# xds0112/5G_based_System_level_Integrated_Sensing_and_Communication_Simulator

Hardware: AMD Instinct MI355X
Metric: sensing slots/sec (CDL echo->2D-FFT->2D-CFAR) (higher is better)
Workload: dtype f64

## Files before the change

### 5g_based_system_level_integrated_sensing_and_communication_simulator_amd/csrc/cov.hip

```cpp
#include <algorithm>
#include <type_traits>
#include "isac_internal.hpp"
#include "echo_dev.hpp"

namespace isac {

typedef double v4f64 __attribute__((ext_vector_type(4)));


constexpr int kCovSyncSlabs = 8;
template <int NB>
struct CovPlan {
  static constexpr int kTiles = NB * (NB + 1) / 2;
  static constexpr int kGroups = (kTiles + 4) / 5;
  static constexpr int kPerGroup = (kTiles + kGroups - 1) / kGroups;
  static constexpr int kPhases = 4 / kGroups;
  static constexpr int kSamplesPerLane = 4 / kPhases;
  static constexpr int first_tile(int grp) { return grp * kPerGroup; }
  static constexpr int tiles_of(int grp) { return first_tile(grp) + kPerGroup <= kTiles ? kPerGroup : kTiles - first_tile(grp); }
};

constexpr int cov_tile_i(int nb, int t) {
  int i = 0;
  while (t >= nb - i) { t -= nb - i; ++i; }
// ... 610 lines not shown
  unsigned long long seed;
  int K, L_whole, L_out, A;
  int s_col;
};
constexpr int kLazyPieces = 19;
__host__ __device__ constexpr int lazy_piece_gap(int i) {
  return (i * 30) / kLazyPieces;
}

template <int QT>
struct CovLazyGenerator {
  static constexpr int NB = 4;
  static constexpr int kGaps = 30;
  struct Cur { int l, sc; long long g; };
  int gp, ga, K, s_col, g_lds0;
  double sig;
  uint32_t key0, key1;
  long long s_end;
  c64 st[2][QT];
  bool ant_ok[2];
  uint64_t colbase[2];
  __amdgpu_buffer_rsrc_t rsD[QT];
  Cur cg, cd;
  uint32_t pc[2][4];
  float wf[2][2][2];
  bool v_half[2];
  c64 dl[2][QT][2];
  __device__ __forceinline__ CovLazyGenerator(const LazyCovArgs& a, long long s_begin, long long s_end_)
      : gp(threadIdx.x & 7), ga(threadIdx.x >> 3), K(a.K), s_col(a.s_col), sig(a.sig), key0((uint32_t)a.seed), key1((uint32_t)(a.seed >> 32)), s_end(s_end_) {
#pragma unroll
    for (int j = 0; j < 2; ++j) {
      const int ant = ga + 32 * j;
      ant_ok[j] = ant < a.A;
      colbase[j] = (uint64_t)a.L_out * (uint64_t)ant;
#pragma unroll
      for (int q = 0; q < QT; ++q) st[j][q] = ant_ok[j] ? a.steer_rq[(long long)ant * QT + q] : mk(0.0, 0.0);
    }
#pragma unroll
    for (int q = 0; q < QT; ++q) rsD[q] = buffer_of(a.D + (long long)q * K * a.L_whole, (unsigned)((long long)K * a.L_whole * (long long)sizeof(c64)));
    g_lds0 = (ga >> 4) * kCovSlabBlk + gp * kCovPitch + ((ga & 15) ^ kCovSwizzle(gp));
    cg = cd = cur_at(s_begin);
  }
  __device__ __forceinline__ Cur cur_at(long long g) const {
    Cur c; c.g = g; c.l = (int)((unsigned)g / (unsigned)s_col); c.sc = (int)((unsigned)g - (unsigned)c.l * (unsigned)s_col); return c;
  }
  __device__ __forceinline__ void advance(Cur& c) const { ++c.g; if (++c.sc == s_col) { c.sc = 0; ++c.l; } }
  __device__ __forceinline__ int k0_of(const Cur& c) const { return ((c.sc >> 6) << 10) + ((c.sc & 63) << 3) + gp; }
  __device__ __forceinline__ void init(const Cur& c) {
    const int k0 = k0_of(c);
    const bool in = c.g < s_end;
    v_half[0] = in && k0 < K;
    v_half[1] = in && k0 + 512 < K;
    const uint32_t slot = (uint32_t)(((c.sc >> 6) << 9) + ((c.sc & 63) << 3) + gp);
#pragma unroll
    for (int j = 0; j < 2; ++j) {
      const uint64_t ctr = (uint64_t)slot + (uint64_t)kSpectralSlotsPerColumn * ((uint64_t)c.l + colbase[j]);
      pc[j][0] = (uint32_t)ctr; pc[j][1] = (uint32_t)(ctr >> 32); pc[j][2] = kSpectralStream; pc[j][3] = 0u;
    }
  }
  template <int R>
  __device__ __forceinline__ void round() {
#pragma unroll
    for (int j = 0; j < 2; ++j) philox4x32_round(pc[j], key0 + (uint32_t)R * 0x9E3779B9u, key1 + (uint32_t)R * 0xBB67AE85u);
  }
  template <int I>
  __device__ __forceinline__ void bm() {
    constexpr int j = I / 2, h = I % 2;
    box_muller32_hw_f32(pc[j][2 * h], pc[j][2 * h + 1], wf[j][h][0], wf[j][h][1]);
  }
  template <int I>
  __device__ __forceinline__ void emit(const c64 (&dv)[QT][2], c64* img) {
    constexpr int j = I / 2, h = I % 2;
    c64 d[QT];
#pragma unroll
    for (int q = 0; q < QT; ++q) d[q] = dv[q][h];
    c64 v = spectral_echo_value<QT, true>(d, st[j], mk((double)wf[j][h][0], (double)wf[j][h][1]), sig);
    const bool ok = v_half[h] && ant_ok[j];
    v = mk(ok ? v.re : 0.0, ok ? v.im : 0.0);
    img[g_lds0 + 2 * j * kCovSlabBlk + 8 * h * kCovPitch] = v;
  }
  __device__ __forceinline__ void loads(c64 (&dv)[QT][2], const Cur& c) {
    const int k0 = k0_of(c);
    const bool in = c.g < s_end;
    const unsigned base = (unsigned)(((long long)K * c.l + k0) * (long long)sizeof(c64));
    const unsigned o0 = (in && k0 < K) ? base : kCovOobOffset, o1 = (in && k0 + 512 < K) ? base + 512u * (unsigned)sizeof(c64) : kCovOobOffset;
#pragma unroll
    for (int q = 0; q < QT; ++q) { dv[q][0] = buffer_load_c64(rsD[q], o0); dv[q][1] = buffer_load_c64(rsD[q], o1); }
  }
  __device__ __forceinline__ void whole(c64 (&dv)[QT][2], c64* img) {
// ... 294 lines not shown
```

### 5g_based_system_level_integrated_sensing_and_communication_simulator_amd/csrc/echo.hip

```cpp
#include <cstring>
#include <type_traits>

#include "isac_internal.hpp"
#include "fft_lds.hpp"
#include "echo_dev.hpp"

namespace isac {

template <int QT, int UNROLL>
__global__ __launch_bounds__(256) void beamsum_kernel(const c64* __restrict__ tx, long long T, int A,
                                                      const c64* __restrict__ steer ,
                                                      c64* __restrict__ beam ) {
  extern __shared__ __attribute__((aligned(16))) char smem_raw[];
  c64* s_steer = reinterpret_cast<c64*>(smem_raw);
  for (int i = threadIdx.x; i < A * QT; i += blockDim.x) s_steer[i] = steer[i];
  __syncthreads();
  for (long long t0 = (long long)blockIdx.x * 256; t0 < T; t0 += (long long)gridDim.x * 256) {
    const long long t = t0 + threadIdx.x;
    const long long tc = t < T ? t : T - 1;
    c64 acc[QT];
#pragma unroll
    for (int q = 0; q < QT; ++q) acc[q] = mk(0.0, 0.0);
    const c64* p = tx + tc;
    int a = 0;
    for (; a + UNROLL <= A; a += UNROLL) {
      c64 v[UNROLL];
#pragma unroll
      for (int u = 0; u < UNROLL; ++u) v[u] = p[(long long)(a + u) * T];
#pragma unroll
      for (int u = 0; u < UNROLL; ++u)
#pragma unroll
        for (int q = 0; q < QT; ++q) acc[q] = fma(v[u], s_steer[q * A + a + u], acc[q]);
    }
    for (; a < A; ++a) {
      c64 v = p[(long long)a * T];
#pragma unroll
      for (int q = 0; q < QT; ++q) acc[q] = fma(v, s_steer[q * A + a], acc[q]);
    }
    if (t < T) {
#pragma unroll
      for (int q = 0; q < QT; ++q) beam[(long long)q * T + t] = acc[q];
    }
  }
}

struct TargetDesc {
  double wd;
  double lsf;
  long long shift;
};
constexpr int kMaxTargets = 64;
struct TargetTable {
  TargetDesc t[kMaxTargets];
};

__global__ __launch_bounds__(256) void coef_kernel(const c64* __restrict__ beam, long long T, int Q,
                                                   TargetTable tab, double w , double Ts,
                                                   c64* __restrict__ coef ,
                                                   c64* __restrict__ phase_rx ) {
  long long t = (long long)blockIdx.x * blockDim.x + threadIdx.x;
  if (t >= T) return;
  double tt = (double)t * Ts;
  double s, c;
  sincos(w * tt, &s, &c);
  c64 prx = mk(c, -s);
  phase_rx[t] = prx;
  for (int q = 0; q < Q; ++q) {
    long long d = tab.t[q].shift;
    c64 out = mk(0.0, 0.0);
    if (t >= d) {
      double sd, cd, st, ct;
      sincos(tab.t[q].wd * tt, &sd, &cd);
      sincos(w * ((double)(t - d) * Ts), &st, &ct);
      c64 v = beam[(long long)q * T + (t - d)] * mk(ct, st);
      v = v * mk(cd, sd);
      v = v * tab.t[q].lsf;
      out = v * prx;
    }
    coef[(long long)q * T + t] = out;
  }
}

__global__ __launch_bounds__(256) void radar_waveform_kernel(long long T, int A, int Q, const c64* __restrict__ coef,
                                                             const c64* __restrict__ steer_rq ,
                                                             const c64* __restrict__ phase_rx, int noise_mode,
                                                             const c64* __restrict__ noise, double n0s, uint64_t seed,
                                                             c64* __restrict__ rx) {
  long long t = (long long)blockIdx.x * blockDim.x + threadIdx.x;
  int r = blockIdx.y;
  if (t >= T) return;
  rx[t + T * r] = rx_sample(t, r, T, Q, coef, steer_rq + (long long)r * Q, phase_rx, noise_mode, noise, n0s, seed);
}

struct OfdmGeom {
  int nfft, n_sc, cp_base, cp_long, sym_per_half;
};

template <class FFT, bool SYNTH, int QT = 0>
__global__ __launch_bounds__(256, 2) void demod_kernel(OfdmGeom g, long long T, int A, int L_whole, int L_out,
                                                       const c64* __restrict__ tw,
                                                       int Q_rt, const c64* __restrict__ coef,
                                                       const c64* __restrict__ steer_rq, const c64* __restrict__ phase_rx,
                                                       int noise_mode, const c64* __restrict__ noise, double n0s,
                                                       uint64_t seed,
                                                       const c64* __restrict__ wave,
                                                       c64* __restrict__ grid, const c64* __restrict__ logtab_g) {
  extern __shared__ __attribute__((aligned(16))) char smem_raw[];
  c64* lds = reinterpret_cast<c64*>(smem_raw);
  const int tid = threadIdx.x;
  FFT fft;
  constexpr bool kTables = SYNTH && QT > 0 && std::is_same<FFT, Fft4096>::value;
  const int Q = QT ? QT : Q_rt;
// ... 127 lines not shown
template <int QT, int NZ, bool STORE = true, int GROUP = (QT <= 1 ? 4 : 2)>
__global__ __launch_bounds__(Fft4096W::NT, kEchoRangeWavesPerSimd) void echo_range_sl_kernel(int K, int L_whole, int L_out, int A, const c64* D,
                                                            const c64* __restrict__ steer_rq, double sig, uint64_t seed,
                                                            const c64* noise, const c64* __restrict__ tw,
                                                            c64* grid,
                                                            const c64* txg, const double* win_k,
                                                            const double* __restrict__ win_r, double inv_n, double sqrt_n,
                                                            int row_lo, int n_rows, c64* __restrict__ ymid) {
  static_assert(QT >= 1 && QT <= 2, "compile-time target count");
  extern __shared__ __attribute__((aligned(16))) char smem_raw[];
  c64* lds = reinterpret_cast<c64*>(smem_raw);
  using FFT = Fft4096W;
  constexpr int NT = FFT::NT, PER = FFT::PER, NG = PER / GROUP;
  const int tid = threadIdx.x;
  FFT fft;
  int l, r;
  if (!spectral_tile_map(blockIdx.x, L_whole, A, l, r)) return;
  const long long colg = (long long)l + (long long)L_out * r;
  const c64* Dl = D + (long long)K * l;
  const long long d_stride = (long long)K * L_whole;
  const c64* ptx = txg + (long long)K * colg;
  const c64* nzc = NZ == 2 ? noise + (long long)K * colg : nullptr;
  const __amdgpu_buffer_rsrc_t rs_dst = buffer_of(grid + (long long)K * colg, (unsigned)K * (unsigned)sizeof(c64));
  c64 s[QT];
#pragma unroll
  for (int q = 0; q < QT; ++q) s[q] = steer_rq[(long long)r * QT + q];
  struct Ld { c64 tx; double w; c64 d[QT]; c64 nz; };
  Ld ld[2][GROUP];
  auto load_group = [&](int g, int b) {
#pragma unroll
    for (int u = 0; u < GROUP; ++u) {
      const int k = tid + NT * (g * GROUP + u);
      const int kc = k < K ? k : K - 1;
      Ld& e = ld[b][u];
      e.tx = ptx[kc];
      e.w = win_k[kc];
      if constexpr (NZ == 2) e.nz = nzc[kc];
#pragma unroll
      for (int q = 0; q < QT; ++q) e.d[q] = Dl[(long long)q * d_stride + kc];
    }
    asm volatile("" ::: "memory");
  };
  fft.init_table(lds, tw, tid);
  load_group(0, 0);
  __builtin_amdgcn_sched_barrier(0);
#pragma unroll
  for (int j = 0; j < PER; ++j) fft.x[j] = mk(0.0, 0.0);
  const int wave_k0 = __builtin_amdgcn_readfirstlane(tid & ~63);
  auto draw = [&](int c) {
    if constexpr (NZ == 1) {
      const int j0 = 2 * c, j1 = j0 + 1;
      if (wave_k0 + NT * j0 < K) {
        const uint64_t ctr = (uint64_t)(tid + NT * c) + (uint64_t)kSpectralSlotsPerColumn * (uint64_t)colg;
        uint32_t o[4];
        philox4x32_10((uint32_t)ctr, (uint32_t)(ctr >> 32), kSpectralStream, 0u, (uint32_t)seed, (uint32_t)(seed >> 32), o);
        fft.x[j0] = box_muller32_hw(o[0], o[1]);
        if (wave_k0 + NT * j1 < K) fft.x[j1] = box_muller32_hw(o[2], o[3]);
      }
    }
  };
  bool live = false;
  auto consume = [&](int g, int b) {
#pragma unroll
    for (int u = 0; u < GROUP; ++u) {
      const int j = g * GROUP + u, k = tid + NT * j;
      const Ld& e = ld[b][u];
      const c64 v = spectral_echo_value<QT, NZ != 0>(e.d, s, NZ == 2 ? e.nz : fft.x[j], sig);
      if constexpr (STORE) buffer_store_c64_nt(rs_dst, (unsigned)k * (unsigned)sizeof(c64), v);
      else asm volatile("" ::"v"(v.re), "v"(v.im) : "memory");
      c64 y = mul_conj(v, e.tx) * e.w;
      y = k < K ? y : mk(0.0, 0.0);
      live |= (y.re != 0.0) | (y.im != 0.0);
      fft.x[j] = y;
    }
  };
#pragma unroll
  for (int g = 0; g < NG; ++g) {
#pragma unroll
    for (int c = g * GROUP / 2; c < (g + 1) * GROUP / 2; ++c) draw(c);
    __builtin_amdgcn_sched_barrier(0);
    if (g + 1 < NG) load_group(g + 1, (g + 1) & 1);
    consume(g, g & 1);
    __builtin_amdgcn_sched_barrier(0);
  }
  c64* yd = ymid + (long long)n_rows * colg;
  if (!__syncthreads_or(live)) {
    for (int rr = tid; rr < n_rows; rr += NT) yd[rr] = mk(0.0, 0.0);
    return;
  }
  fft.init_twiddles_lds(lds, tid);
  const int blk = FFT::block_of_rows(row_lo, n_rows);
  fft.template transform<+1>(lds, tw, tid, blk);
  auto put = [&](int n, c64 v) {
    const int rr = n - row_lo;
    const double wr = win_r[n];
    if (rr >= 0 && rr < n_rows) yd[rr] = ((v * inv_n) * sqrt_n) * wr;
  };
  if (blk >= 0) fft.drain_block(put, tid, blk);
  else fft.drain(put, tid);
}

struct ModIo {
  long long wave_rows, t_off;
  int grid_cols, l_off, sym0, n_win;
// ... 91 lines not shown
  if (c->scs_khz != 15 && c->scs_khz != 30 && c->scs_khz != 60 && c->scs_khz != 120)
    return fail(ctx, ISAC_ERR_INVALID_ARG, "carrier.scs_khz must be 15/30/60/120");
  return ISAC_OK;
}

static OfdmGeom geom_of(const isac_carrier* c) {
  Numerology n = numerology(c->nfft, c->scs_khz);
  return OfdmGeom{c->nfft, c->n_sc, n.cp_base, n.cp_long, n.sym_per_half};
}

static int whole_symbols(const OfdmGeom& g, long long T) {
  long long lo = 0, hi = T / g.nfft + 1;
  while (lo < hi) {
    long long mid = (lo + hi + 1) / 2;
    if (symbol_start((int)mid, g.nfft, g.cp_base, g.cp_long, g.sym_per_half) <= T) lo = mid; else hi = mid - 1;
  }
  return (int)lo;
}

extern "C" int isac_ofdm_symbol_count(const isac_carrier* carrier, int64_t T, int32_t* n_symbols) {
  if (!carrier || !n_symbols || T < 0) return ISAC_ERR_INVALID_ARG;
  *n_symbols = whole_symbols(geom_of(carrier), T);
  return ISAC_OK;
}

extern "C" int isac_ofdm_waveform_length(const isac_carrier* carrier, int32_t L, int64_t* T) {
  if (!carrier || !T || L < 0) return ISAC_ERR_INVALID_ARG;
  OfdmGeom g = geom_of(carrier);
  *T = symbol_start(L, g.nfft, g.cp_base, g.cp_long, g.sym_per_half);
  return ISAC_OK;
}

static int prepare_echo(isac_ctx* ctx, const c64* d_tx, long long T, const isac_radar_channel_params* rp,
                        const uint8_t* los, int* q_out) {
  if (!d_tx || !rp || !los) return fail(ctx, ISAC_ERR_INVALID_ARG, "NULL argument");
  if (T <= 0 || rp->n_ants <= 0 || rp->n_targets < 0) return fail(ctx, ISAC_ERR_INVALID_ARG, "bad T / n_ants / n_targets");
  ctx->lazy.valid = false;
  if (!(rp->fs > 0)) return fail(ctx, ISAC_ERR_INVALID_ARG, "fs must be positive");
  const int A = rp->n_ants;
  const double c0 = 299792458.0;
  const double lambda = c0 / rp->fc;
  const double Ts = 1.0 / rp->fs;
  const double two_pi = 2.0 * M_PI;
  TargetTable tab{};
  std::vector<c64> steer_aq;
  int Q = 0;
  for (int i = 0; i < rp->n_targets; ++i) {
    if (los[i] != 1) continue;
    if (Q >= kMaxTargets) return fail(ctx, ISAC_ERR_CAPACITY, "more than 64 LoS targets");
    for (int a = 0; a < A; ++a) {
      const isac_c64 sv = rp->rx_steering[(size_t)a + (size_t)A * i];
      steer_aq.push_back(mk(sv.re, sv.im));
    }
    double path_delay = 2.0 * rp->range[i] / c0;
    tab.t[Q].shift = (long long)std::ceil(path_delay / Ts);
    double fd = 2.0 * rp->velocity[i] / lambda;
    tab.t[Q].wd = two_pi * fd;
    tab.t[Q].lsf = rp->large_scale_fading[i];
    ++Q;
  }
  if (Q == 0) return fail(ctx, ISAC_ERR_NO_LOS, "no LoS target: rxWaveform is empty (basicRadarChannel.m:59,64)");
  std::vector<c64> steer_rq((size_t)A * Q);
  for (int q = 0; q < Q; ++q)
    for (int a = 0; a < A; ++a) steer_rq[(size_t)a * Q + q] = steer_aq[(size_t)q * A + a];
  ISAC_TRY(ensure(ctx, ctx->steer, sizeof(c64) * (size_t)A * Q * 2));
  ISAC_TRY(ensure(ctx, ctx->beam, sizeof(c64) * (size_t)Q * T));
  ISAC_TRY(ensure(ctx, ctx->coef, sizeof(c64) * (size_t)Q * T));
  ISAC_TRY(ensure(ctx, ctx->phase_rx, sizeof(c64) * (size_t)T));
  c64* d_steer_aq = (c64*)ctx->steer.p;
  {
    const size_t bytes = sizeof(c64) * (size_t)A * Q * 2;
    void* hst = nullptr;
    ISAC_TRY(stage_acquire(ctx, bytes, &hst));
    std::memcpy(hst, steer_aq.data(), bytes / 2);
    std::memcpy((char*)hst + bytes / 2, steer_rq.data(), bytes / 2);
    ISAC_TRY(stage_commit(ctx, d_steer_aq, bytes));
  }
  const unsigned gb = cdiv(T, 256);
  const unsigned gbs = (unsigned)std::min<long long>(gb, 1024);
  timeline_mark(ctx, 0, ctx->stream);
#define ISAC_BEAMSUM(QT) \
  hipLaunchKernelGGL((beamsum_kernel<QT, (QT <= 2 ? 32 : 8)>), dim3(gbs), dim3(256), sizeof(c64) * A * QT, ctx->stream, d_tx, T, A, st, bm)
  for (int q0 = 0; q0 < Q;) {
    int rem = Q - q0;
    const c64* st = d_steer_aq + (size_t)q0 * A;
    c64* bm = (c64*)ctx->beam.p + (size_t)q0 * T;
    if (rem >= 8) { ISAC_BEAMSUM(8); q0 += 8; }
    else if (rem >= 4) { ISAC_BEAMSUM(4); q0 += 4; }
    else if (rem >= 2) { ISAC_BEAMSUM(2); q0 += 2; }
    else { ISAC_BEAMSUM(1); q0 += 1; }
  }
#undef ISAC_BEAMSUM
  timeline_mark(ctx, 1, ctx->stream);
  const double w = two_pi * rp->fc;
  hipLaunchKernelGGL(coef_kernel, dim3(gb), dim3(256), 0, ctx->stream, (const c64*)ctx->beam.p, T, Q, tab, w, Ts,
                     (c64*)ctx->coef.p, (c64*)ctx->phase_rx.p);
  ISAC_HIP(hipGetLastError());
  *q_out = Q;
  return ISAC_OK;
}

extern "C" int isac_basic_radar_channel_dev(isac_ctx* ctx, const isac_c64* d_tx_wave, int64_t T,
                                            const isac_radar_channel_params* rp, const uint8_t* los, int noise_mode,
                                            const isac_c64* d_noise_unit, uint64_t seed, isac_c64* d_rx_wave) {
  ISAC_ENTER(ctx);
  if (!d_rx_wave) return fail(ctx, ISAC_ERR_INVALID_ARG, "rx_wave is NULL");
  if (noise_mode == ISAC_NOISE_INJECTED && !d_noise_unit) return fail(ctx, ISAC_ERR_INVALID_ARG, "noise buffer missing");
  if (noise_mode < ISAC_NOISE_NONE || noise_mode > ISAC_NOISE_PHILOX)
    return fail(ctx, ISAC_ERR_INVALID_ARG, "basicRadarChannel returns a time-domain waveform: noise modes NONE / INJECTED / PHILOX only");
  int Q = 0;
  ISAC_TRY(prepare_echo(ctx, (const c64*)d_tx_wave, T, rp, los, &Q));
  const int A = rp->n_ants;
  const double n0s = std::sqrt(rp->n0 / 2.0);
  hipLaunchKernelGGL(radar_waveform_kernel, dim3(cdiv(T, 256), A), dim3(256), 0, ctx->stream, (long long)T, A, Q,
                     (const c64*)ctx->coef.p, (const c64*)ctx->steer.p + (size_t)A * Q, (const c64*)ctx->phase_rx.p,
                     noise_mode, (const c64*)d_noise_unit, n0s, seed, (c64*)d_rx_wave);
  ISAC_HIP(hipGetLastError());
  return ISAC_OK;
}

template <int MAXQ, class F>
static int echo_dispatch(int Q, F&& f) {
  if constexpr (MAXQ > 0)
    if (Q != MAXQ) return echo_dispatch<MAXQ - 1>(Q, f);
  return f(std::integral_constant<int, MAXQ>{});
}

static int padded_symbols(int L_whole, int tx_dim_l, int32_t* l_out) {
  const int L_out = L_whole < tx_dim_l ? tx_dim_l : L_whole;
  if (l_out) *l_out = L_out;
  return L_out;
}

template <class FFT, bool SYNTH, int QT = 0>
static int launch_demod(isac_ctx* ctx, const OfdmGeom& g, long long T, int A, int L_whole, int L_out, const c64* tw, int Q,
                        int noise_mode, const c64* noise, double n0s, uint64_t seed, const c64* wave, c64* grid) {
  size_t lds = sizeof(c64) * (FFT::LDS_ELEMS + kLogTabSize);
  const c64* logtab = nullptr;
  ISAC_TRY(isac_get_logtab(ctx, &logtab));
  auto kern = demod_kernel<FFT, SYNTH, QT>;
  ISAC_TRY(allow_lds(ctx, reinterpret_cast<const void*>(kern), lds));
  hipLaunchKernelGGL(kern, dim3((unsigned)(L_whole * A)) , dim3(256), lds, ctx->stream, g, T, A, L_whole, L_out, tw, Q,
                     (const c64*)ctx->coef.p, SYNTH ? (const c64*)ctx->steer.p + (size_t)A * Q : nullptr,
                     (const c64*)ctx->phase_rx.p, noise_mode, noise, n0s, seed, wave, grid, logtab);
  ISAC_HIP(hipGetLastError());
  return ISAC_OK;
}

static int spectral_prepare(isac_ctx* ctx, const c64* d_tx, long long T, const isac_radar_channel_params* rp, const uint8_t* los,
                            const OfdmGeom& g, int* q_out, int* l_whole_out) {
  int Q = 0;
  ISAC_TRY(prepare_echo(ctx, d_tx, T, rp, los, &Q));
  const int L_whole = whole_symbols(g, T);
  if (L_whole <= 0) return fail(ctx, ISAC_ERR_SHORT_WAVEFORM, "waveform shorter than one OFDM symbol");
  ISAC_TRY(ensure(ctx, ctx->dgrid, sizeof(c64) * (size_t)g.n_sc * L_whole * Q));
  const c64* tw = nullptr;
  ISAC_TRY(isac_get_twiddles(ctx, g.nfft, &tw));
  ISAC_FFT_DISPATCH(g.nfft, ISAC_TRY((launch_demod<FFT, false>(ctx, g, T, Q, L_whole, L_whole, tw, 0, 0, nullptr, 0.0, 0,
                                                               (const c64*)ctx->coef.p, (c64*)ctx->dgrid.p))));
  *q_out = Q;
  *l_whole_out = L_whole;
  return ISAC_OK;
}

static bool spectral_mode(int noise_mode) { return noise_mode == ISAC_NOISE_PHILOX_SPECTRAL || noise_mode == ISAC_NOISE_INJECTED_SPECTRAL; }

template <int QT>
static int launch_echo_spectral(isac_ctx* ctx, const OfdmGeom& g, int A, int L_whole, int L_out, int Q, int noise_mode,
                                const c64* noise, double sig, uint64_t seed, c64* grid) {
  const dim3 gr((unsigned)spectral_grid_size(L_whole, A)), bl(256);
  const c64* D = (const c64*)ctx->dgrid.p;
  const c64* srq = (const c64*)ctx->steer.p + (size_t)A * Q;
  auto kern = noise_mode == ISAC_NOISE_PHILOX_SPECTRAL ? echo_spectral_kernel<QT, 1> : noise_mode == ISAC_NOISE_INJECTED_SPECTRAL ? echo_spectral_kernel<QT, 2> : echo_spectral_kernel<QT, 0>;
  hipLaunchKernelGGL(kern, gr, bl, 0, ctx->stream, g.n_sc, L_whole, L_out, A, Q, D, srq, sig, seed, noise, grid);
  ISAC_HIP(hipGetLastError());
  return ISAC_OK;
}

template <class Kern, class... Args>
static int launch_echo_range(isac_ctx* ctx, Kern kern, int L_whole, int A, Args... args) {
  const size_t lds = sizeof(c64) * Fft4096W::LDS_ELEMS;
  ISAC_TRY(allow_lds(ctx, reinterpret_cast<const void*>(kern), lds));
  hipLaunchKernelGGL(kern, dim3((unsigned)spectral_grid_size(L_whole, A)), dim3(Fft4096W::NT), lds, ctx->stream, args...);
  ISAC_HIP(hipGetLastError());
  return ISAC_OK;
// ... 61 lines not shown
  OfdmGeom g = geom_of(carrier);
  CutRows cr;
  const bool rows_ok = cut_rows_ok(ep, cf, &cr) && cf->row1 >= cf->row0;
  const bool fusable = g.nfft == 4096 && ep->n_ifft == g.nfft && rows_ok;
  const bool lazy = d_echo_grid == nullptr;
  bool lazy_native = false;
  if (lazy) {
    int n_los = 0;
    if (!los) return fail(ctx, ISAC_ERR_INVALID_ARG, "NULL argument");
    for (int i = 0; i < rp->n_targets; ++i) n_los += los[i] == 1;
    lazy_native = fusable && noise_mode == ISAC_NOISE_PHILOX_SPECTRAL && rp->n_ants > 48 && rp->n_ants <= 64 && n_los >= 1 && n_los <= 2;
    if (!lazy_native) {
      int32_t lw = 0;
      ISAC_TRY(isac_ofdm_symbol_count(carrier, T, &lw));
      const int lo_ = padded_symbols(lw, tx_dim_l, nullptr);
      if (lo_ <= 0) return fail(ctx, ISAC_ERR_SHORT_WAVEFORM, "waveform shorter than one OFDM symbol");
      ISAC_TRY(ensure(ctx, ctx->echo_own, sizeof(c64) * (size_t)g.n_sc * lo_ * rp->n_ants));
      d_echo_grid = (isac_c64*)ctx->echo_own.p;
    }
  }
  auto plain_then_range = [&](bool cache_rows) -> int {
    int32_t lo = 0;
    ISAC_TRY(isac_mono_static_sensing_dev(ctx, d_tx_wave, T, tx_dim_l, carrier, rp, los, noise_mode, d_noise_unit, seed, d_echo_grid, &lo));
    if (l_out) *l_out = lo;
    if (lazy) ctx->lazy.set_owned(g.n_sc, lo, rp->n_ants);
    if (!cache_rows) return ISAC_OK;
    return isac_range_stage_into_cache(ctx, ep, cf, (const c64*)d_echo_grid, (const c64*)d_tx_grid, g.n_sc, lo, rp->n_ants);
  };
  if (!fusable) return plain_then_range(rows_ok && ep->n_ifft >= g.n_sc && (ep->n_ifft & (ep->n_ifft - 1)) == 0);
  if (noise_mode < ISAC_NOISE_NONE || noise_mode > ISAC_NOISE_INJECTED_SPECTRAL) return fail(ctx, ISAC_ERR_INVALID_ARG, "unknown noise mode");
  if (noise_mode == ISAC_NOISE_INJECTED_SPECTRAL && !d_noise_unit) return fail(ctx, ISAC_ERR_INVALID_ARG, "noise buffer missing");
  if (!spectral_mode(noise_mode)) return plain_then_range(true);
  int Q = 0, L_whole = 0;
  ISAC_TRY(spectral_prepare(ctx, (const c64*)d_tx_wave, T, rp, los, g, &Q, &L_whole));
  const int A = rp->n_ants, row_lo = cr.row_lo, nr = cr.nr;
  const int L_out = padded_symbols(L_whole, tx_dim_l, l_out);
  ctx->tgt.drop();
  ISAC_TRY(ensure(ctx, ctx->ymid, sizeof(c64) * (size_t)nr * L_out * A));
  if (L_out > L_whole) {
    if (!lazy_native) ISAC_HIP(hipMemsetAsync(d_echo_grid, 0, sizeof(c64) * (size_t)g.n_sc * L_out * A, ctx->stream));
    ISAC_HIP(hipMemsetAsync(ctx->ymid.p, 0, sizeof(c64) * (size_t)nr * L_out * A, ctx->stream));
  }
  const c64* tw = nullptr;
  const double *wk = nullptr, *wr = nullptr;
  ISAC_TRY(isac_get_w512_pack(ctx, &tw));
  ISAC_TRY(isac_get_windows(ctx, g.n_sc, ep->n_ifft, &wk, &wr));
  const double sig = std::sqrt(rp->n0 / 2.0) * std::sqrt((double)g.nfft);
  if (!ctx->profile_cov) ISAC_TRY(profile_begin(ctx));
  timeline_mark(ctx, 2, ctx->stream);
  auto launch = [&](auto kern, auto... q_rt) {
    return launch_echo_range(ctx, kern, L_whole, A, g.n_sc, L_whole, L_out, A, q_rt..., (const c64*)ctx->dgrid.p, (const c64*)ctx->steer.p + (size_t)A * Q, sig, seed,
                             (const c64*)d_noise_unit, tw, (c64*)d_echo_grid, (const c64*)d_tx_grid, wk, wr, 1.0 / ep->n_ifft, std::sqrt((double)ep->n_ifft), row_lo, nr,
                             (c64*)ctx->ymid.p);
  };
  const bool philox = noise_mode == ISAC_NOISE_PHILOX_SPECTRAL;
  ISAC_TRY(echo_dispatch<4>(Q, [&](auto qc) {
    constexpr int QT = decltype(qc)::value;
    if constexpr (QT == 1 || QT == 2)
      return launch(lazy_native ? echo_range_sl_kernel<QT, 1, false> : philox ? echo_range_sl_kernel<QT, 1> : echo_range_sl_kernel<QT, 2>);
    else
      return launch(philox ? echo_range_kernel<QT, 1> : echo_range_kernel<QT, 2>, Q);
  }));
  if (!ctx->profile_cov) ISAC_TRY(profile_end(ctx));
  timeline_mark(ctx, 3, ctx->stream);
  ctx->range_cache.set(d_echo_grid, d_tx_grid, g.n_sc, L_out, A, ep->n_ifft, row_lo, nr);
  if (lazy_native) ctx->lazy.set_native(g.n_sc, L_whole, L_out, A, Q, sig, seed);
  else if (lazy) ctx->lazy.set_owned(g.n_sc, L_out, A);
// ... 128 lines not shown
```

### 5g_based_system_level_integrated_sensing_and_communication_simulator_amd/csrc/echo_dev.hpp

```cpp
#pragma once
#include "isac_common.hpp"

namespace isac {

__device__ __forceinline__ void philox4x32_10(uint32_t c0, uint32_t c1, uint32_t c2, uint32_t c3,
                                              uint32_t k0, uint32_t k1, uint32_t (&out)[4]) {
#pragma unroll
  for (int r = 0; r < 10; ++r) {
    uint64_t p0 = (uint64_t)0xD2511F53u * c0;
    uint64_t p1 = (uint64_t)0xCD9E8D57u * c2;
    uint32_t hi0 = (uint32_t)(p0 >> 32), lo0 = (uint32_t)p0;
    uint32_t hi1 = (uint32_t)(p1 >> 32), lo1 = (uint32_t)p1;
    uint32_t n0 = hi1 ^ c1 ^ k0, n2 = hi0 ^ c3 ^ k1;
    c0 = n0; c1 = lo1; c2 = n2; c3 = lo0;
    k0 += 0x9E3779B9u;
    k1 += 0xBB67AE85u;
  }
  out[0] = c0; out[1] = c1; out[2] = c2; out[3] = c3;
}

__device__ __forceinline__ double ln_unit(double u) {
  int e;
  double m = frexp(u, &e);
  if (m < 0.70710678118654752440) { m *= 2.0; --e; }
  const double d = m + 1.0;
  double rc = __builtin_amdgcn_rcp(d);
  rc = rc * ::fma(-d, rc, 2.0);
  rc = rc * ::fma(-d, rc, 2.0);
  const double t = (m - 1.0) * rc, t2 = t * t;
  double p = 1.0 / 19.0;
  p = ::fma(p, t2, 1.0 / 17.0); p = ::fma(p, t2, 1.0 / 15.0); p = ::fma(p, t2, 1.0 / 13.0); p = ::fma(p, t2, 1.0 / 11.0);
  p = ::fma(p, t2, 1.0 / 9.0);  p = ::fma(p, t2, 1.0 / 7.0);  p = ::fma(p, t2, 1.0 / 5.0);  p = ::fma(p, t2, 1.0 / 3.0);
  p = ::fma(p, t2, 1.0);
  return ::fma((double)e, 0.69314718055994530942, 2.0 * t * p);
}

__device__ __forceinline__ double sqrt_neg2log(double u) {
  const double y = -2.0 * ln_unit(u);
  if (!(y > 0.0)) return 0.0;
  double rs = __builtin_amdgcn_rsq(y);
  double sq = y * rs;
  double h = 0.5 * rs;
  double res = ::fma(-sq, sq, y);
  sq = ::fma(res, h, sq);
  res = ::fma(-sq, sq, y);
  sq = ::fma(res, h, sq);
// ... 45 lines not shown
  const int i = (int)(hi >> 24);
  const double rem = ::fma((double)(hi & 0x00FFFFFFu), 2097152.0, (double)(o[2] >> 11));
  const double phi = rem * (6.28318530717958647692 * 0x1.0p-53);
  const double p2 = phi * phi;
  const double sphi = phi * ::fma(p2, ::fma(p2, ::fma(p2, -1.0 / 5040.0, 1.0 / 120.0), -1.0 / 6.0), 1.0);
  const double cphi = ::fma(p2, ::fma(p2, ::fma(p2, -1.0 / 720.0, 1.0 / 24.0), -0.5), 1.0);
  const c64 w = w256[i];
  const double c = ::fma(w.re, cphi, w.im * sphi);
  const double sn = ::fma(w.re, sphi, -w.im * cphi);
  return c64{rad * c, rad * sn};
}

constexpr uint32_t kSpectralStream = 2u;
constexpr int kSpectralSlotsPerColumn = 2048;

__device__ __forceinline__ c64 box_muller32_hw(uint32_t ur, uint32_t ua) {
  const float u = __builtin_fmaf((float)ur, 0x1.0p-32f, 0x1.0p-33f);
  const float rad = __builtin_amdgcn_sqrtf(__builtin_amdgcn_logf(u) * -1.3862943611198906f);
  const float turns = (float)ua * 0x1.0p-32f;
  return c64{(double)(rad * __builtin_amdgcn_cosf(turns)), (double)(rad * __builtin_amdgcn_sinf(turns))};
}

__device__ __forceinline__ void box_muller32_hw_f32(uint32_t ur, uint32_t ua, float& re, float& im) {
  const float u = __builtin_fmaf((float)ur, 0x1.0p-32f, 0x1.0p-33f);
  const float rad = __builtin_amdgcn_sqrtf(__builtin_amdgcn_logf(u) * -1.3862943611198906f);
  const float turns = (float)ua * 0x1.0p-32f;
  re = rad * __builtin_amdgcn_cosf(turns);
  im = rad * __builtin_amdgcn_sinf(turns);
}

__device__ __forceinline__ void philox4x32_round(uint32_t (&c)[4], uint32_t k0r, uint32_t k1r) {
  const uint64_t p0 = (uint64_t)0xD2511F53u * c[0];
  const uint64_t p1 = (uint64_t)0xCD9E8D57u * c[2];
  const uint32_t n0 = (uint32_t)(p1 >> 32) ^ c[1] ^ k0r, n2 = (uint32_t)(p0 >> 32) ^ c[3] ^ k1r;
  c[0] = n0; c[1] = (uint32_t)p1; c[2] = n2; c[3] = (uint32_t)p0;
}

template <int QT, bool NOISE>
__device__ __forceinline__ c64 spectral_echo_value(const c64 (&d)[QT], const c64 (&s)[QT], c64 w, double sig) {
  c64 v = mk(0.0, 0.0);
#pragma unroll
  for (int q = 0; q < QT; ++q) v = fma(d[q], s[q], v);
  if constexpr (NOISE) v = v + w * sig;
  return v;
}

constexpr int kTileSyms = 8, kTileAnts = 8;
__host__ __device__ inline int spectral_grid_size(int L_whole, int A) {
  const int n_tiles = ((L_whole + kTileSyms - 1) / kTileSyms) * ((A + kTileAnts - 1) / kTileAnts);
  return ((n_tiles + 7) / 8) * 8 * (kTileSyms * kTileAnts);
}
__device__ __forceinline__ bool spectral_tile_map(int wg, int L_whole, int A, int& l, int& r) {
  const int x = wg & 7, s = wg >> 3;
  const int tile = (s / (kTileSyms * kTileAnts)) * 8 + x, within = s % (kTileSyms * kTileAnts);
  const int n_ag = (A + kTileAnts - 1) / kTileAnts;
  const int ag = tile % n_ag, lb = tile / n_ag;
  r = kTileAnts * ag + within / kTileSyms;
  l = kTileSyms * lb + within % kTileSyms;
  return r < A && l < L_whole;
}

template <int QT, int NZ, int GROUP, int NT, class PRE, class E>
__device__ __forceinline__ void spectral_echo_column(int tid, int K, int Q_rt, const c64* __restrict__ Dl ,
                                                     long long d_stride , const c64* __restrict__ sr ,
                                                     double sig, uint64_t seed, long long column, const c64* __restrict__ nz,
                                                     c64 (&acc)[4096 / NT],
                                                     PRE&& pre, E&& emit) {
// ... 87 lines not shown
```

### 5g_based_system_level_integrated_sensing_and_communication_simulator_amd/csrc/tables.hip

```cpp
#include "isac_internal.hpp"

using namespace isac;

namespace {

double bessel_i0(double x) {
  double q = 0.25 * x * x, term = 1.0, sum = 1.0;
  for (int k = 1; k < 200; ++k) {
    term *= q / ((double)k * (double)k);
    sum += term;
    if (term < 1e-18 * sum) break;
  }
  return sum;
}

std::vector<double> kaiser_window(int n, double beta) {
  std::vector<double> w((size_t)n, 1.0);
  if (n == 1) return w;
  const int odd = n % 2;
  const double xind = (double)(n - 1) * (double)(n - 1);
  const int half = (n + 1) / 2;
  const double den = bessel_i0(std::fabs(beta));
  std::vector<double> h((size_t)half);
  for (int i = 0; i < half; ++i) {
// ... 20 lines not shown
    if (n % 4 == 0) { w[(size_t)n / 4] = mk(0.0, -1.0); w[(size_t)n / 2] = mk(-1.0, 0.0); w[(size_t)3 * n / 4] = mk(0.0, 1.0); }
  });
}

int isac_get_w512_pack(isac_ctx* ctx, const c64** out) {
  return cached_table(ctx, {kW512Pack}, out, [](std::vector<c64>& w) {
    w.resize(520);
    const long double two_pi = 2.0L * 3.14159265358979323846264338327950288L;
    for (int m = 0; m < 512; ++m) { const long double a = -two_pi * (long double)(8 * m) / 4096.0L; w[(size_t)m] = mk((double)cosl(a), (double)sinl(a)); }
    for (int m = 0; m < 8; ++m) { const long double a = -two_pi * (long double)m / 4096.0L; w[(size_t)512 + m] = mk((double)cosl(a), (double)sinl(a)); }
    w[0] = mk(1.0, 0.0); w[128] = mk(0.0, -1.0); w[256] = mk(-1.0, 0.0); w[384] = mk(0.0, 1.0); w[512] = mk(1.0, 0.0);
  });
}

int isac_get_logtab(isac_ctx* ctx, const c64** out) {
  return cached_table(ctx, {kLogTab}, out, [](std::vector<c64>& lt) {
    lt.resize(128);
    for (int i = 0; i < 128; ++i) {
      const long double c = 0.5L * (1.0L + ((long double)i + 0.5L) / 128.0L);
      const double inv = (double)(1.0L / c);
      lt[(size_t)i] = mk(inv, (double)(-logl((long double)inv)));
    }
  });
}

int isac_get_rise_window(isac_ctx* ctx, int n_win, const double** out) {
  return cached_table(ctx, {kRiseWindow, {n_win}}, out, [&](std::vector<double>& w) {
    w.resize((size_t)n_win);
    for (int i = 1; i <= n_win; ++i) w[(size_t)i - 1] = 0.5 * (1.0 - std::sin(M_PI * (n_win + 1 - 2.0 * i) / (2.0 * n_win)));
  });
}

int isac_get_windows(isac_ctx* ctx, int K, int n_ifft, const double** win_k, const double** win_r) {
  auto get = [&](int n, bool shifted, const double** out) {
    return cached_table(ctx, {shifted ? kKaiser3Shifted : kKaiser3, {n}}, out, [&](std::vector<double>& w) {
      w = kaiser_window(n, 3.0);
      if (shifted) {
        std::vector<double> s((size_t)n);
        const int sh = (n + 1) / 2;
        for (int i = 0; i < n; ++i) s[(size_t)i] = w[(size_t)((i + sh) % n)];
        w.swap(s);
      }
    });
  };
  ISAC_TRY(get(K, false, win_k));
  ISAC_TRY(get(n_ifft, true, win_r));
  return ISAC_OK;
}
```

Baseline: 20590.

## Fuse beamsum and coef kernels, pad window, use bitop3 xor in philox

Adds a fused beamsum+coef kernel for Q<=2 in the spectral path. It scatters the coefficient to t=u+shift directly, which removes the beam buffer round trip and one kernel launch. Philox XORs become a single three-input bitop3 instruction, and the per-lane counter math in the covariance generator is hoisted into colbase. The Kaiser window is zero-padded to the FFT length so the k<K masking in the spectral loop can be dropped. In the fused path phase_rx is no longer written and coef now depends on the scattered writes covering every index, so correctness hinges on those coverage assumptions.

New measurement: 21280, median of 6. +3.3%, better.

```diff
diff --git a/5g_based_system_level_integrated_sensing_and_communication_simulator_amd/csrc/cov.hip b/5g_based_system_level_integrated_sensing_and_communication_simulator_amd/csrc/cov.hip
--- a/5g_based_system_level_integrated_sensing_and_communication_simulator_amd/csrc/cov.hip
+++ b/5g_based_system_level_integrated_sensing_and_communication_simulator_amd/csrc/cov.hip
@@ -666,7 +666,7 @@
     for (int j = 0; j < 2; ++j) {
       const int ant = ga + 32 * j;
       ant_ok[j] = ant < a.A;
-      colbase[j] = (uint64_t)a.L_out * (uint64_t)ant;
+      colbase[j] = (uint64_t)gp + (uint64_t)kSpectralSlotsPerColumn * ((uint64_t)a.L_out * (uint64_t)ant);
 #pragma unroll
       for (int q = 0; q < QT; ++q) st[j][q] = ant_ok[j] ? a.steer_rq[(long long)ant * QT + q] : mk(0.0, 0.0);
     }
@@ -685,10 +685,11 @@
     const bool in = c.g < s_end;
     v_half[0] = in && k0 < K;
     v_half[1] = in && k0 + 512 < K;
-    const uint32_t slot = (uint32_t)(((c.sc >> 6) << 9) + ((c.sc & 63) << 3) + gp);
+    const uint32_t slot = (uint32_t)(((c.sc >> 6) << 9) + ((c.sc & 63) << 3));
+    const uint64_t slab = (uint64_t)slot + (uint64_t)kSpectralSlotsPerColumn * (uint64_t)c.l;
 #pragma unroll
     for (int j = 0; j < 2; ++j) {
-      const uint64_t ctr = (uint64_t)slot + (uint64_t)kSpectralSlotsPerColumn * ((uint64_t)c.l + colbase[j]);
+      const uint64_t ctr = slab + colbase[j];
       pc[j][0] = (uint32_t)ctr; pc[j][1] = (uint32_t)(ctr >> 32); pc[j][2] = kSpectralStream; pc[j][3] = 0u;
     }
   }
diff --git a/5g_based_system_level_integrated_sensing_and_communication_simulator_amd/csrc/echo.hip b/5g_based_system_level_integrated_sensing_and_communication_simulator_amd/csrc/echo.hip
--- a/5g_based_system_level_integrated_sensing_and_communication_simulator_amd/csrc/echo.hip
+++ b/5g_based_system_level_integrated_sensing_and_communication_simulator_amd/csrc/echo.hip
@@ -6,6 +6,27 @@
 #include "echo_dev.hpp"
 
 namespace isac {
+
+template <int QT, int UNROLL>
+__device__ __forceinline__ void beam_sample(const c64* __restrict__ p , long long T, int A, const c64* __restrict__ s_steer , c64 (&acc)[QT]) {
+#pragma unroll
+  for (int q = 0; q < QT; ++q) acc[q] = mk(0.0, 0.0);
+  int a = 0;
+  for (; a + UNROLL <= A; a += UNROLL) {
+    c64 v[UNROLL];
+#pragma unroll
+    for (int u = 0; u < UNROLL; ++u) v[u] = p[(long long)(a + u) * T];
+#pragma unroll
+    for (int u = 0; u < UNROLL; ++u)
+#pragma unroll
+      for (int q = 0; q < QT; ++q) acc[q] = fma(v[u], s_steer[q * A + a + u], acc[q]);
+  }
+  for (; a < A; ++a) {
+    c64 v = p[(long long)a * T];
+#pragma unroll
+    for (int q = 0; q < QT; ++q) acc[q] = fma(v, s_steer[q * A + a], acc[q]);
+  }
+}
 
 template <int QT, int UNROLL>
 __global__ __launch_bounds__(256) void beamsum_kernel(const c64* __restrict__ tx, long long T, int A,
@@ -19,24 +40,7 @@
     const long long t = t0 + threadIdx.x;
     const long long tc = t < T ? t : T - 1;
     c64 acc[QT];
-#pragma unroll
-    for (int q = 0; q < QT; ++q) acc[q] = mk(0.0, 0.0);
-    const c64* p = tx + tc;
-    int a = 0;
-    for (; a + UNROLL <= A; a += UNROLL) {
-      c64 v[UNROLL];
-#pragma unroll
-      for (int u = 0; u < UNROLL; ++u) v[u] = p[(long long)(a + u) * T];
-#pragma unroll
-      for (int u = 0; u < UNROLL; ++u)
-#pragma unroll
-        for (int q = 0; q < QT; ++q) acc[q] = fma(v[u], s_steer[q * A + a + u], acc[q]);
-    }
-    for (; a < A; ++a) {
-      c64 v = p[(long long)a * T];
-#pragma unroll
-      for (int q = 0; q < QT; ++q) acc[q] = fma(v, s_steer[q * A + a], acc[q]);
-    }
+    beam_sample<QT, UNROLL>(tx + tc, T, A, s_steer, acc);
     if (t < T) {
 #pragma unroll
       for (int q = 0; q < QT; ++q) beam[(long long)q * T + t] = acc[q];
@@ -54,6 +58,22 @@
   TargetDesc t[kMaxTargets];
 };
 
+__device__ __forceinline__ c64 rx_phase(double w , double tt) {
+  double s, c;
+  sincos(w * tt, &s, &c);
+  return mk(c, -s);
+}
+
+__device__ __forceinline__ c64 coef_value(c64 b, long long t, const TargetDesc& td, double w, double Ts, double tt, c64 prx) {
+  double sd, cd, st, ct;
+  sincos(td.wd * tt, &sd, &cd);
+  sincos(w * ((double)(t - td.shift) * Ts), &st, &ct);
+  c64 v = b * mk(ct, st);
+  v = v * mk(cd, sd);
+  v = v * td.lsf;
+  return v * prx;
+}
+
 __global__ __launch_bounds__(256) void coef_kernel(const c64* __restrict__ beam, long long T, int Q,
                                                    TargetTable tab, double w , double Ts,
                                                    c64* __restrict__ coef ,
@@ -61,23 +81,44 @@
   long long t = (long long)blockIdx.x * blockDim.x + threadIdx.x;
   if (t >= T) return;
   double tt = (double)t * Ts;
-  double s, c;
-  sincos(w * tt, &s, &c);
-  c64 prx = mk(c, -s);
+  c64 prx = rx_phase(w, tt);
   phase_rx[t] = prx;
   for (int q = 0; q < Q; ++q) {
     long long d = tab.t[q].shift;
     c64 out = mk(0.0, 0.0);
-    if (t >= d) {
-      double sd, cd, st, ct;
-      sincos(tab.t[q].wd * tt, &sd, &cd);
-      sincos(w * ((double)(t - d) * Ts), &st, &ct);
-      c64 v = beam[(long long)q * T + (t - d)] * mk(ct, st);
-      v = v * mk(cd, sd);
-      v = v * tab.t[q].lsf;
-      out = v * prx;
+    if (t >= d) out = coef_value(beam[(long long)q * T + (t - d)], t, tab.t[q], w, Ts, tt, prx);
+    coef[(long long)q * T + t] = out;
+  }
+}
+
+template <int QT>
+struct CoefTargets {
+  TargetDesc t[QT];
+};
+template <int QT, int UNROLL>
+__global__ __launch_bounds__(256) void beamsum_coef_kernel(const c64* __restrict__ tx, long long T, int A,
+                                                           const c64* __restrict__ steer ,
+                                                           CoefTargets<QT> tab, double w , double Ts,
+                                                           c64* __restrict__ coef ) {
+  extern __shared__ __attribute__((aligned(16))) char smem_raw[];
+  c64* s_steer = reinterpret_cast<c64*>(smem_raw);
+  for (int i = threadIdx.x; i < A * QT; i += blockDim.x) s_steer[i] = steer[i];
+  __syncthreads();
+  for (long long t0 = (long long)blockIdx.x * 256; t0 < T; t0 += (long long)gridDim.x * 256) {
+    const long long u = t0 + threadIdx.x;
+    const long long uc = u < T ? u : T - 1;
+    c64 acc[QT];
+    beam_sample<QT, UNROLL>(tx + uc, T, A, s_steer, acc);
+#pragma unroll
+    for (int q = 0; q < QT; ++q) {
+      const long long d = tab.t[q].shift, t = u + d;
+      c64* cq = coef + (long long)q * T;
+      if (u < d && u < T) cq[u] = mk(0.0, 0.0);
+      if (u < T && t >= 0 && t < T) {
+        const double tt = (double)t * Ts;
+        cq[t] = coef_value(acc[q], t, tab.t[q], w, Ts, tt, rx_phase(w, tt));
+      }
     }
-    coef[(long long)q * T + t] = out;
   }
 }
 
@@ -271,12 +312,14 @@
     for (int u = 0; u < GROUP; ++u) {
       const int k = tid + NT * (g * GROUP + u);
       const int kc = k < K ? k : K - 1;
+      const unsigned o16 = (unsigned)kc * (unsigned)sizeof(c64);
+      auto at = [](const auto* base, unsigned off) { return *reinterpret_cast<decltype(base)>(reinterpret_cast<const char*>(base) + off); };
       Ld& e = ld[b][u];
-      e.tx = ptx[kc];
-      e.w = win_k[kc];
-      if constexpr (NZ == 2) e.nz = nzc[kc];
-#pragma unroll
-      for (int q = 0; q < QT; ++q) e.d[q] = Dl[(long long)q * d_stride + kc];
+      e.tx = at(ptx, o16);
+      e.w = at(win_k, (unsigned)k * (unsigned)sizeof(double));
+      if constexpr (NZ == 2) e.nz = at(nzc, o16);
+#pragma unroll
+      for (int q = 0; q < QT; ++q) e.d[q] = at(Dl + (long long)q * d_stride, o16);
     }
     asm volatile("" ::: "memory");
   };
@@ -307,8 +350,7 @@
       const c64 v = spectral_echo_value<QT, NZ != 0>(e.d, s, NZ == 2 ? e.nz : fft.x[j], sig);
       if constexpr (STORE) buffer_store_c64_nt(rs_dst, (unsigned)k * (unsigned)sizeof(c64), v);
       else asm volatile("" ::"v"(v.re), "v"(v.im) : "memory");
-      c64 y = mul_conj(v, e.tx) * e.w;
-      y = k < K ? y : mk(0.0, 0.0);
+      const c64 y = mul_conj(v, e.tx) * e.w;
       live |= (y.re != 0.0) | (y.im != 0.0);
       fft.x[j] = y;
     }
@@ -466,7 +508,7 @@
 }
 
 static int prepare_echo(isac_ctx* ctx, const c64* d_tx, long long T, const isac_radar_channel_params* rp,
-                        const uint8_t* los, int* q_out) {
+                        const uint8_t* los, int* q_out, bool coef_only = false) {
   if (!d_tx || !rp || !los) return fail(ctx, ISAC_ERR_INVALID_ARG, "NULL argument");
   if (T <= 0 || rp->n_ants <= 0 || rp->n_targets < 0) return fail(ctx, ISAC_ERR_INVALID_ARG, "bad T / n_ants / n_targets");
   ctx->lazy.valid = false;
@@ -513,6 +555,21 @@
   const unsigned gb = cdiv(T, 256);
   const unsigned gbs = (unsigned)std::min<long long>(gb, 1024);
   timeline_mark(ctx, 0, ctx->stream);
+  const double w = two_pi * rp->fc;
+  if (coef_only && Q <= 2) {
+    auto launch = [&](auto qc) {
+      constexpr int QT = decltype(qc)::value;
+      CoefTargets<QT> ct;
+      for (int q = 0; q < QT; ++q) ct.t[q] = tab.t[q];
+      hipLaunchKernelGGL((beamsum_coef_kernel<QT, 32>), dim3(gbs), dim3(256), sizeof(c64) * A * QT, ctx->stream, d_tx, T, A, (const c64*)d_steer_aq, ct, w, Ts, (c64*)ctx->coef.p);
+    };
+    if (Q == 1) launch(std::integral_constant<int, 1>{});
+    else launch(std::integral_constant<int, 2>{});
+    ISAC_HIP(hipGetLastError());
+    timeline_mark(ctx, 1, ctx->stream);
+    *q_out = Q;
+    return ISAC_OK;
+  }
 #define ISAC_BEAMSUM(QT) \
   hipLaunchKernelGGL((beamsum_kernel<QT, (QT <= 2 ? 32 : 8)>), dim3(gbs), dim3(256), sizeof(c64) * A * QT, ctx->stream, d_tx, T, A, st, bm)
   for (int q0 = 0; q0 < Q;) {
@@ -526,7 +583,6 @@
   }
 #undef ISAC_BEAMSUM
   timeline_mark(ctx, 1, ctx->stream);
-  const double w = two_pi * rp->fc;
   hipLaunchKernelGGL(coef_kernel, dim3(gb), dim3(256), 0, ctx->stream, (const c64*)ctx->beam.p, T, Q, tab, w, Ts,
                      (c64*)ctx->coef.p, (c64*)ctx->phase_rx.p);
   ISAC_HIP(hipGetLastError());
@@ -582,9 +638,9 @@
 }
 
 static int spectral_prepare(isac_ctx* ctx, const c64* d_tx, long long T, const isac_radar_channel_params* rp, const uint8_t* los,
-                            const OfdmGeom& g, int* q_out, int* l_whole_out) {
+                            const OfdmGeom& g, int* q_out, int* l_whole_out, bool coef_only = false) {
   int Q = 0;
-  ISAC_TRY(prepare_echo(ctx, d_tx, T, rp, los, &Q));
+  ISAC_TRY(prepare_echo(ctx, d_tx, T, rp, los, &Q, coef_only));
   const int L_whole = whole_symbols(g, T);
   if (L_whole <= 0) return fail(ctx, ISAC_ERR_SHORT_WAVEFORM, "waveform shorter than one OFDM symbol");
   ISAC_TRY(ensure(ctx, ctx->dgrid, sizeof(c64) * (size_t)g.n_sc * L_whole * Q));
@@ -712,7 +768,7 @@
   if (noise_mode == ISAC_NOISE_INJECTED_SPECTRAL && !d_noise_unit) return fail(ctx, ISAC_ERR_INVALID_ARG, "noise buffer missing");
   if (!spectral_mode(noise_mode)) return plain_then_range(true);
   int Q = 0, L_whole = 0;
-  ISAC_TRY(spectral_prepare(ctx, (const c64*)d_tx_wave, T, rp, los, g, &Q, &L_whole));
+  ISAC_TRY(spectral_prepare(ctx, (const c64*)d_tx_wave, T, rp, los, g, &Q, &L_whole, true));
   const int A = rp->n_ants, row_lo = cr.row_lo, nr = cr.nr;
   const int L_out = padded_symbols(L_whole, tx_dim_l, l_out);
   ctx->tgt.drop();
diff --git a/5g_based_system_level_integrated_sensing_and_communication_simulator_amd/csrc/echo_dev.hpp b/5g_based_system_level_integrated_sensing_and_communication_simulator_amd/csrc/echo_dev.hpp
--- a/5g_based_system_level_integrated_sensing_and_communication_simulator_amd/csrc/echo_dev.hpp
+++ b/5g_based_system_level_integrated_sensing_and_communication_simulator_amd/csrc/echo_dev.hpp
@@ -2,6 +2,14 @@
 #include "isac_common.hpp"
 
 namespace isac {
+
+__device__ __forceinline__ uint32_t xor3(uint32_t a, uint32_t b, uint32_t c) {
+#if defined(__HIP_DEVICE_COMPILE__) && __has_builtin(__builtin_amdgcn_bitop3_b32)
+  return __builtin_amdgcn_bitop3_b32(a, b, c, 0x96);
+#else
+  return a ^ b ^ c;
+#endif
+}
 
 __device__ __forceinline__ void philox4x32_10(uint32_t c0, uint32_t c1, uint32_t c2, uint32_t c3,
                                               uint32_t k0, uint32_t k1, uint32_t (&out)[4]) {
@@ -11,7 +19,7 @@
     uint64_t p1 = (uint64_t)0xCD9E8D57u * c2;
     uint32_t hi0 = (uint32_t)(p0 >> 32), lo0 = (uint32_t)p0;
     uint32_t hi1 = (uint32_t)(p1 >> 32), lo1 = (uint32_t)p1;
-    uint32_t n0 = hi1 ^ c1 ^ k0, n2 = hi0 ^ c3 ^ k1;
+    uint32_t n0 = xor3(hi1, c1, k0), n2 = xor3(hi0, c3, k1);
     c0 = n0; c1 = lo1; c2 = n2; c3 = lo0;
     k0 += 0x9E3779B9u;
     k1 += 0xBB67AE85u;
@@ -123,7 +131,7 @@
 __device__ __forceinline__ void philox4x32_round(uint32_t (&c)[4], uint32_t k0r, uint32_t k1r) {
   const uint64_t p0 = (uint64_t)0xD2511F53u * c[0];
   const uint64_t p1 = (uint64_t)0xCD9E8D57u * c[2];
-  const uint32_t n0 = (uint32_t)(p1 >> 32) ^ c[1] ^ k0r, n2 = (uint32_t)(p0 >> 32) ^ c[3] ^ k1r;
+  const uint32_t n0 = xor3((uint32_t)(p1 >> 32), c[1], k0r), n2 = xor3((uint32_t)(p0 >> 32), c[3], k1r);
   c[0] = n0; c[1] = (uint32_t)p1; c[2] = n2; c[3] = (uint32_t)p0;
 }
 
diff --git a/5g_based_system_level_integrated_sensing_and_communication_simulator_amd/csrc/tables.hip b/5g_based_system_level_integrated_sensing_and_communication_simulator_amd/csrc/tables.hip
--- a/5g_based_system_level_integrated_sensing_and_communication_simulator_amd/csrc/tables.hip
+++ b/5g_based_system_level_integrated_sensing_and_communication_simulator_amd/csrc/tables.hip
@@ -76,8 +76,8 @@
 }
 
 int isac_get_windows(isac_ctx* ctx, int K, int n_ifft, const double** win_k, const double** win_r) {
-  auto get = [&](int n, bool shifted, const double** out) {
-    return cached_table(ctx, {shifted ? kKaiser3Shifted : kKaiser3, {n}}, out, [&](std::vector<double>& w) {
+  auto get = [&](int n, int n_pad, bool shifted, const double** out) {
+    return cached_table(ctx, {shifted ? kKaiser3Shifted : kKaiser3, {n, n_pad}}, out, [&](std::vector<double>& w) {
       w = kaiser_window(n, 3.0);
       if (shifted) {
         std::vector<double> s((size_t)n);
@@ -85,9 +85,10 @@
         for (int i = 0; i < n; ++i) s[(size_t)i] = w[(size_t)((i + sh) % n)];
         w.swap(s);
       }
+      if (n_pad > n) w.resize((size_t)n_pad, 0.0);
     });
   };
-  ISAC_TRY(get(K, false, win_k));
-  ISAC_TRY(get(n_ifft, true, win_r));
+  ISAC_TRY(get(K, K > n_ifft ? K : n_ifft, false, win_k));
+  ISAC_TRY(get(n_ifft, n_ifft, true, win_r));
   return ISAC_OK;
 }
```
